# MariaPdg/thesis-fmri-reconstruction

Measured on NVIDIA B200. Metric: stage1_vaegan_train_samples_per_sec_64x64, higher is better.
Workload: dtype bf16

## Files before the change

thesis_fmri_reconstruction_b200/csrc/api.cu:

```cuda
#include <cstdarg>
#include <cstdio>
#include <cstring>
#include <cstdlib>
#include <algorithm>

#include "../../include/fmri_b200.h"
#include "simt_kernels.cuh"
#include "tc_kernels.cuh"
#include "hconv_kernels.cuh"
#include "hwgrad_kernels.cuh"
#include "cto3_kernels.cuh"
#include "mmd_kernels.cuh"
#include "eval_kernels.cuh"
#include "similarity_kernels.cuh"

using namespace fmri;

static thread_local char g_err[512] = "";
static int fail(int code, const char* fmt, ...) {
    va_list ap;
    va_start(ap, fmt);
    vsnprintf(g_err, sizeof(g_err), fmt, ap);
    va_end(ap);
    return code;
// ... 486 lines not shown
    c.num_taps = 1;
    c.lim_x = M;
    c.lim_y = 1;
    c.out_off = 0;
    c.taps[0].map = 0;
    c.taps[0].dx = 0;
    c.taps[0].dy = 0;
    c.taps[0].brow = 0;
    p.num_chunks = cdiv(K, KCH);
    p.n_total = N;
    p.n_tiles = N / BN;
    const int splits = 1;
    p.splits = splits;
    p.a_bytes = p.bw * KCH * 2;
    p.out_sn = 0;
    p.out_sy = 0;
    p.out_sx = ldc;
    p.out = Cout;
    p.out_fp32 = c_fp32;
    p.atomic_out = (splits > 1 || accumulate) ? 1 : 0;
    if (p.atomic_out && !c_fp32) return fail(FMRI_ERR_ARG, "accumulating gemm needs fp32 output");
    p.bias = bias;
    p.act = act;
    return dispatch_ig(p, BN, KCH, 1, st);
}

template <int BN, int NCH, int STAGES, int TG>
static int launch_wg(const WgParams& p, cudaStream_t st) {
    using L = WgSmem<BN, NCH, STAGES, TG>;
    static bool attr_done = false;
    if (!attr_done) {
        CUDA_OK(cudaFuncSetAttribute(wgrad_kernel<BN, NCH, STAGES, TG>, cudaFuncAttributeMaxDynamicSharedMemorySize,
                                     L::TOTAL));
        attr_done = true;
    }
    dim3 grid(cdiv(p.num_taps, TG), p.m_tiles * p.n_tiles, p.splits);
    wgrad_kernel<BN, NCH, STAGES, TG><<<grid, 192, L::TOTAL, st>>>(p);
    LAUNCH_OK();
    return 0;
}
static int wave_splits(long long base, long long max_splits) {
    const long long lo = std::max<long long>(1, (148 + base - 1) / base);
    if (max_splits <= lo) return (int)std::max<long long>(1, max_splits);
    const long long hi = std::min<long long>(max_splits, std::max<long long>(lo, (3 * 148) / base));
    long long best = lo;
    double best_score = -1.0;
    for (long long s = lo; s <= hi; ++s) {
        const long long ctas = base * s, waves = (ctas + 147) / 148;
        const double score = (double)ctas / (148.0 * waves) - 0.01 * waves;
        if (score > best_score) { best_score = score; best = s; }
    }
    return (int)best;
}
static int dispatch_wg(const WgParams& p, int BN, int NCH, cudaStream_t st) {
    if (NCH == 64 && BN == 128) return p.num_taps > 1 ? launch_wg<128, 64, 2, 2>(p, st) : launch_wg<128, 64, 3, 1>(p, st);
    if (NCH == 64 && BN == 64) return launch_wg<64, 64, 4, 1>(p, st);
    if (NCH == 32 && BN == 32) return p.num_taps % 5 == 0 ? launch_wg<32, 32, 3, 5>(p, st) : launch_wg<32, 32, 4, 1>(p, st);
    return fail(FMRI_ERR_UNSUPPORTED, "wgrad tile BN=%d NCH=%d not instantiated", BN, NCH);
}
static int run_wgrad_tc(const void* Dn, int N, int PH, int PW, int Cd, const void* Sh, int BH, int BW, int Cs,
                        int stride, int num_taps, float* ws, cudaStream_t st) {
    if (Cd % 64 || Cs % 32) return fail(FMRI_ERR_UNSUPPORTED, "wgrad tensor path needs Cd%%64==0, Cs%%32==0");
    WgParams p;
    memset(&p, 0, sizeof(p));
    pick_box(PW, PH, N, &p.bw, &p.bh, &p.bn);
    if ((p.bw * p.bh * p.bn) % 16) pick_box_pow2(PW, PH, N, &p.bw, &p.bh, &p.bn);
    p.rows = p.bw * p.bh * p.bn;
    if (p.rows % 16) return fail(FMRI_ERR_UNSUPPORTED, "wgrad pixel box %d not a multiple of 16", p.rows);
    p.tiles_x = cdiv(PW, p.bw);
    p.tiles_y = cdiv(PH, p.bh);
    p.tiles_n = cdiv(N, p.bn);
    const int NCH = (Cs % 64 == 0) ? 64 : 32;
    const int BN = (Cs % 128 == 0) ? 128 : (Cs % 64 == 0 ? 64 : 32);
    if (NCH == 32 && BN != 32) return fail(FMRI_ERR_UNSUPPORTED, "wgrad Cs=%d", Cs);
    int rc = make_act_map(&p.mapD, Dn, Cd, PW, PH, N, Cd, (long long)PW * Cd, (long long)PH * PW * Cd, 64, p.bw,
                          p.bh, p.bn);
    if (rc) return rc;
    const __nv_bfloat16* sb = reinterpret_cast<const __nv_bfloat16*>(Sh);
    if (stride == 2) {
        for (int ph = 0; ph < 2; ++ph)
            for (int pw = 0; pw < 2; ++pw) {
                const int Wp = (BW - pw + 1) / 2, Hp = (BH - ph + 1) / 2;
                rc = make_act_map(&p.mapS[ph * 2 + pw], sb + ((long long)ph * BW + pw) * Cs, Cs, Wp, Hp, N, 2LL * Cs,
                                  2LL * BW * Cs, (long long)BH * BW * Cs, NCH, p.bw, p.bh, p.bn);
                if (rc) return rc;
            }
    } else {
        rc = make_act_map(&p.mapS[0], sb, Cs, BW, BH, N, Cs, (long long)BW * Cs, (long long)BH * BW * Cs, NCH, p.bw,
                          p.bh, p.bn);
        if (rc) return rc;
    }
    p.num_taps = num_taps;
    for (int kh = 0; kh < 5; ++kh)
        for (int kw = 0; kw < 5; ++kw) {
            TapDesc& t = p.taps[kh * 5 + kw];
            if (num_taps == 1) {
                t.map = 0;
                t.dx = t.dy = 0;
            } else if (stride == 2) {
                t.map = (int16_t)((kh & 1) * 2 + (kw & 1));
                t.dy = (int16_t)((kh - 2 - (kh & 1)) / 2);
                t.dx = (int16_t)((kw - 2 - (kw & 1)) / 2);
            } else {
                t.map = 0;
                t.dy = (int16_t)(kh - 2);
                t.dx = (int16_t)(kw - 2);
            }
        }
    p.m_total = Cd;
    p.n_total = Cs;
    p.m_tiles = cdiv(Cd, 128);
    p.n_tiles = Cs / BN;
    const long long pt = (long long)p.tiles_x * p.tiles_y * p.tiles_n;
    const int tap_groups = (NCH == 32 && BN == 32 && num_taps % 5 == 0) ? num_taps / 5
                           : ((NCH == 64 && BN == 128 && num_taps > 1) ? (num_taps + 1) / 2 : num_taps);
    const long long base = (long long)tap_groups * p.m_tiles * p.n_tiles;
    p.splits = wave_splits(base, std::max<long long>(1, pt / 4));
    const long long n = (long long)num_taps * Cd * Cs;
    SCRATCH(slices, float, (long long)p.splits * n, st);
    CUDA_OK(cudaMemsetAsync(slices, 0, sizeof(float) * (size_t)p.splits * n, st));
    p.out = slices;
    p.split_stride = n;
    rc = dispatch_wg(p, BN, NCH, st);
    if (rc) return rc;
    rc = ordered_add(slices, p.splits, n, ws, st);
    CUDA_OK(cudaFreeAsync(slices, st));
    return rc;
}

extern "C" void fmri_conv_out_hw(const fmri_conv_desc* d, int* OH, int* OW) {
    if (d->transposed) {
        *OH = 2 * d->H - 1 + d->output_pad;
        *OW = 2 * d->W - 1 + d->output_pad;
    } else {
        *OH = (d->H - 1) / d->stride + 1;
        *OW = (d->W - 1) / d->stride + 1;
    }
}
static int check_conv(const fmri_conv_desc* d) {
    if (!d || d->N <= 0 || d->H <= 0 || d->W <= 0 || d->Cin <= 0 || d->Cout <= 0)
        return fail(FMRI_ERR_ARG, "bad conv descriptor");
    if (d->stride != 1 && d->stride != 2) return fail(FMRI_ERR_ARG, "conv stride must be 1 or 2");
    if (d->transposed && d->stride != 2) return fail(FMRI_ERR_ARG, "ConvTranspose2d is stride 2 only");
    if (d->dtype != FMRI_F32 && d->dtype != FMRI_BF16) return fail(FMRI_ERR_ARG, "bad dtype");
    return 0;
}
static inline long long w_so(const fmri_conv_desc* d) { return d->transposed ? 25LL : 25LL * d->Cin; }
static inline long long w_si(const fmri_conv_desc* d) { return d->transposed ? 25LL * d->Cout : 25LL; }

extern "C" size_t fmri_conv_pack_elems(const fmri_conv_desc* d) {
    size_t n = 25 * (size_t)d->Cin * d->Cout;
    const int thin = d->transposed ? d->Cout : d->Cin;
    const int other = d->transposed ? d->Cin : d->Cout;
    if (thin == 32 && d->stride == 2) n += 9 * 128 * (size_t)other;
    return n;
}

extern "C" int fmri_conv_pack_weights(const fmri_conv_desc* d, const float* w, void* pack_f, void* pack_d,
                                      void* stream) {
    int rc = check_conv(d);
    if (rc) return rc;
    const long long n = 25LL * d->Cin * d->Cout;
    if (pack_f) {
        permute4_kernel<float, __nv_bfloat16><<<grid1d(n, 256), 256, 0, S(stream)>>>(
            w, reinterpret_cast<__nv_bfloat16*>(pack_f), 1, 25, d->Cout, d->Cin, 0, 1, w_so(d), w_si(d), 0);
        LAUNCH_OK();
        if (d->transposed && d->Cout == 32 && d->stride == 2) {
            __nv_bfloat16* pk = reinterpret_cast<__nv_bfloat16*>(pack_f);
            merge_pack_kernel<<<grid1d(9LL * 128 * d->Cin, 256), 256, 0, S(stream)>>>(pk, pk + n, d->Cin);
            LAUNCH_OK();
        }
    }
    if (pack_d) {
        permute4_kernel<float, __nv_bfloat16><<<grid1d(n, 256), 256, 0, S(stream)>>>(
            w, reinterpret_cast<__nv_bfloat16*>(pack_d), 1, 25, d->Cin, d->Cout, 0, 1, w_si(d), w_so(d), 0);
        LAUNCH_OK();
// ... 142 lines not shown
    p.accumulate = accumulate;
    const float *A, *B;
    if (!d->transposed) {
        A = reinterpret_cast<const float*>(dy); p.PH = OH; p.PW = OW; p.Ca = d->Cout;
        B = reinterpret_cast<const float*>(x); p.BH = d->H; p.BW = d->W; p.Cb = d->Cin;
    } else {
        A = reinterpret_cast<const float*>(x); p.PH = d->H; p.PW = d->W; p.Ca = d->Cin;
        B = reinterpret_cast<const float*>(dy); p.BH = OH; p.BW = OW; p.Cb = d->Cout;
    }
    p.a_sn = (long long)p.PH * p.PW * p.Ca; p.a_sy = (long long)p.PW * p.Ca; p.a_sx = p.Ca; p.a_sc = 1;
    p.b_sn = (long long)p.BH * p.BW * p.Cb; p.b_sy = (long long)p.BW * p.Cb; p.b_sx = p.Cb; p.b_sc = 1;
    p.w_sa = 25LL * p.Cb;
    p.w_sb = 25;
    direct_wgrad_kernel<float, float><<<25 * p.Ca * p.Cb, 128, 0, S(stream)>>>(A, B, dw, p);
    LAUNCH_OK();
    return 0;
}

static const size_t HC_WS_PACK = 65536;
extern "C" size_t fmri_edge_workspace(const fmri_edge_desc* d) {
    return std::max(sizeof(float) * 75 * (size_t)d->C, HC_WS_PACK + (size_t)d->N * d->H * d->W * 16);
}

static bool hc_build(HcParams& p, HcPackSpec& spec, int N, int H, int W, int chunks, int stride, int OH, int OW, int BN,
                     bool flip) {
    memset(&p, 0, sizeof(p));
    memset(&spec, 0, sizeof(spec));
    p.N = N; p.H = H; p.W = W; p.chunks = chunks; p.OH = OH; p.OW = OW;
    const int hx = stride == 1 ? 4 : 2;
    if (stride == 1) {
        p.num_planes = 1;
        p.pl_ys[0] = p.pl_xs[0] = 1;
        p.pl_yoff[0] = p.pl_xoff[0] = -2;
    } else {
        p.num_planes = 4;
        for (int ph = 0; ph < 2; ++ph)
            for (int pw = 0; pw < 2; ++pw) {
                const int pl = ph * 2 + pw;
                p.pl_ys[pl] = p.pl_xs[pl] = 2;
                p.pl_yoff[pl] = ph - 2;
                p.pl_xoff[pl] = pw - 2;
            }
    }
    p.PW = OW + hx;
    if (p.PW > 200) return false;
    const int max_off = hx * p.PW + hx;
    const int nsteps = chunks >= 2 ? 25 * (chunks / 2) : 13;
    if (nsteps > HC_MAX_STEPS) return false;
    p.num_steps = nsteps;
    bool found = false;
    for (int pass = 0; pass < 2 && !found; ++pass) {
        const int mt_max = std::min(5, (pass == 0 ? 128 : 256) / BN);
        const size_t smem_cap = pass == 0 ? 110 * 1024 : 227 * 1024;
        double best = 0.0;
        for (int tht = std::min(OH, (mt_max * 128) / p.PW); tht >= 1; --tht) {
            HcParams q = p;
            q.THt = tht;
            q.tiles_y = cdiv(OH, tht);
            q.MT = cdiv((long long)tht * q.PW, 128);
            q.PH = tht + hx;
            q.slab_rows = (q.PH * q.PW + 7) / 8 * 8 + (chunks > 1 ? 2 : 0);
            const long long overshoot = ((long long)q.MT * 128 + max_off + 1 - q.slab_rows) * 16;
            if (overshoot > 0 && overshoot > hc_b_bytes(q, BN)) continue;
            if ((size_t)hc_smem_bytes(q, BN) > smem_cap) continue;
            const double eff = (double)OH * OW / ((double)q.tiles_y * q.MT * 128);
            if (eff > best + 1e-9) { best = eff; p = q; found = true; }
        }
    }
    if (!found) return false;
    int woff[25];
    for (int kh = 0; kh < 5; ++kh)
        for (int kw = 0; kw < 5; ++kw) {
            int plane = 0, dyr = kh, dxr = kw;
            if (stride == 2) {
                plane = (kh & 1) * 2 + (kw & 1);
                dyr = (kh - 2 - (kh & 1)) / 2 + 1;
                dxr = (kw - 2 - (kw & 1)) / 2 + 1;
            }
            woff[kh * 5 + kw] = plane * chunks * p.slab_rows + dyr * p.PW + dxr;
        }
    int s = 0;
    if (chunks >= 2) {
        for (int tp = 0; tp < 25; ++tp)
            for (int j = 0; j < chunks / 2; ++j, ++s) {
                p.steps[s].a_off = woff[tp] + 2 * j * p.slab_rows;
                p.steps[s].a_lbo = p.slab_rows;
                p.steps[s].b_off = s * BN;
                spec.tap[s][0] = spec.tap[s][1] = (int16_t)(flip ? 24 - tp : tp);
                spec.cb[s][0] = (int16_t)(16 * j);
                spec.cb[s][1] = (int16_t)(16 * j + 8);
            }
    } else {
        int order[25];
        for (int i = 0; i < 25; ++i) order[i] = i;
        std::sort(order, order + 25, [&](int a, int b) { return woff[a] < woff[b]; });
        {
            const int t0 = order[0];
            p.steps[s].a_off = woff[t0];
            p.steps[s].a_lbo = 1;
            p.steps[s].b_off = s * BN;
            spec.tap[s][0] = (int16_t)(flip ? 24 - t0 : t0);
            spec.tap[s][1] = -1;
            spec.cb[s][0] = spec.cb[s][1] = 0;
            ++s;
        }
        for (int i = 1; i < 25; i += 2, ++s) {
            const int t0 = order[i], t1 = order[i + 1];
            p.steps[s].a_off = woff[t0];
            p.steps[s].a_lbo = woff[t1] - woff[t0];
            p.steps[s].b_off = s * BN;
            spec.tap[s][0] = (int16_t)(flip ? 24 - t0 : t0);
            spec.tap[s][1] = (int16_t)(flip ? 24 - t1 : t1);
            spec.cb[s][0] = spec.cb[s][1] = 0;
            if (p.steps[s].a_lbo == 0) return false;
        }
    }
    return true;
}

// ... 35 lines not shown
    }
    return fail(FMRI_ERR_UNSUPPORTED, "hconv BN=%d", BN);
}

static int cto3_run(const void* X, int N, int H, int W, int C, const float* w, long long s_co, long long s_c, int flip,
                    const float* bias, int act, float* img, void* ws, cudaStream_t st) {
    if (C != 32 || W != C3_W || H < 3 || N < 74) return 1;
    C3Params p;
    memset(&p, 0, sizeof(p));
    __nv_bfloat16* wt = reinterpret_cast<__nv_bfloat16*>(ws);
    c3_pack_weights_kernel<<<cdiv(C3_NB * C, 256), 256, 0, st>>>(w, wt, s_co, s_c, flip, C);
    LAUNCH_OK();
    if (make_act_map(&p.mapX, X, C, H * W, 1, N, C, (long long)H * W * C, (long long)H * W * C, C, 128, 1, 1)) return 1;
    {
        const long long dims[2] = {C, C3_NB};
        const long long stv[1] = {C};
        const int box[2] = {C, C3_NB};
        if (make_map(&p.mapW, wt, 2, dims, stv, box, C * 2)) return 1;
    }
    p.N = N; p.H = H; p.out = img; p.bias = bias; p.act = act;
    static bool attr_done = false;
    if (!attr_done) {
        CUDA_OK(cudaFuncSetAttribute(cto3_kernel, cudaFuncAttributeMaxDynamicSharedMemorySize, C3_SMEM));
        attr_done = true;
    }
    cto3_kernel<<<std::min(N, 148), C3_THREADS, C3_SMEM, st>>>(p);
    LAUNCH_OK();
    return 0;
}

static int hconv_c_to_3(const void* X, int N, int H, int W, int C, const float* w, long long s_co, long long s_c, int flip,
                        const float* bias, int act, float* img, void* ws, cudaStream_t st) {
    if (C != 32 && C != 64) return 1;
    {
        const int rc = cto3_run(X, N, H, W, C, w, s_co, s_c, flip, bias, act, img, ws, st);
        if (rc <= 0) return rc;
    }
    HcParams p;
    HcPackSpec spec;
    if (!hc_build(p, spec, N, H, W, C / 8, 1, H, W, 16, flip != 0)) return 1;
    p.X = reinterpret_cast<const __nv_bfloat16*>(X);
    p.epi = 0; p.out = img; p.bias = bias; p.act = act; p.n_out = 3;
    return hc_run(p, spec, 16, w, 3, C, s_co, s_c, ws, st);
}

static int hconv_3_to_c(const float* i0, const float* i1, const float* i2, int nps, int N, int H, int W, int C, int stride,
                        const float* w, long long s_c, long long s_ci, int flip, const float* bias, int act, void* y,
                        void* ws, cudaStream_t st) {
    if (C != 32 && C != 64) return 1;
    const int OH = (H - 1) / stride + 1, OW = (W - 1) / stride + 1;
    HcParams p;
    HcPackSpec spec;
    if (!hc_build(p, spec, N, H, W, 1, stride, OH, OW, C, flip != 0)) return 1;
    __nv_bfloat16* img8 = reinterpret_cast<__nv_bfloat16*>(reinterpret_cast<uint8_t*>(ws) + HC_WS_PACK);
    img8_pack_kernel<<<grid1d((long long)N * H * W, 256), 256, 0, st>>>(i0, i1, i2, nps, N, (long long)H * W, img8);
    LAUNCH_OK();
    p.X = img8;
    p.epi = 1; p.out = y; p.bias = bias; p.act = act; p.n_out = C;
    return hc_run(p, spec, C, w, C, 3, s_c, s_ci, ws, st);
}

static int hwgrad_run(const void* T, const float* i0, const float* i1, const float* i2, int nps, int N, int PH, int PW, int C,
                      float* dwk, float* dbias, int flip, void* ws, cudaStream_t st, int plane = -1, int IH = 0, int IW = 0) {
    if (C != 32 && C != 64) return 1;
    HwParams p;
    memset(&p, 0, sizeof(p));
    p.N = N; p.PH = PH; p.PW = PW; p.C = C;
    p.PWp = (PW + 4 + 15) / 16 * 16;
    if (p.PWp > 128) return 1;
    const int bh_cap = 2;
    p.bh = std::max(1, std::min(std::min(PH, bh_cap), 256 / p.PWp));
    p.tiles_y = cdiv(PH, p.bh);
    p.slab_rows = ((p.bh + 4) * p.PWp + 16 + 7) / 8 * 8;
    p.d_chunk = (p.bh * p.PWp * 128 + 1023) / 1024 * 1024;
    p.stages = 2;
    if (hw_smem_bytes(p) > 227 * 1024) return 1;
    while (p.stages < HW_MAX_STAGES) {
        ++p.stages;
        if (hw_smem_bytes(p) > 110 * 1024) { --p.stages; break; }
    }
    const long long dims[4] = {C, PW, PH, N};
    const long long strides[3] = {C, (long long)PW * C, (long long)PH * PW * C};
    const int box[4] = {64, p.PWp, p.bh, 1};
    if (make_map(&p.mapT, T, 4, dims, strides, box, 128)) return 1;
    __nv_bfloat16* img8 = reinterpret_cast<__nv_bfloat16*>(reinterpret_cast<uint8_t*>(ws) + HC_WS_PACK);
    p.kh0 = 0; p.nkh = 5;
    if (plane < 0) {
        img8_pack_kernel<<<grid1d((long long)N * PH * PW, 256), 256, 0, st>>>(i0, i1, i2, nps, N, (long long)PH * PW, img8);
    } else {
        p.plane = 1; p.ph = plane >> 1; p.pw = plane & 1;
        p.kh0 = 1; p.nkh = p.ph ? 2 : 3;
        img8_plane_pack_kernel<<<grid1d((long long)N * PH * PW, 256), 256, 0, st>>>(i0, i1, i2, nps, N, IH, IW, PH, PW, p.ph,
                                                                                   p.pw, img8);
    }
    LAUNCH_OK();
    p.img8 = img8;
    p.dwk = dwk; p.dbias = dbias; p.flip = flip;
    const int smem = hw_smem_bytes(p);
    static int attr_smem = 0;
    if (smem > attr_smem) {
        CUDA_OK(cudaFuncSetAttribute(hwgrad_kernel, cudaFuncAttributeMaxDynamicSharedMemorySize, smem));
        attr_smem = smem;
    }
    const int total = N * p.tiles_y;
    const int nb = std::min(total, 148 * (smem <= 110 * 1024 ? 2 : 1));
    const long long nw = 75LL * C;
    SCRATCH(part, float, (long long)nb * (nw + C), st);
    CUDA_OK(cudaMemsetAsync(part, 0, sizeof(float) * (size_t)nb * (nw + C), st));
    p.dwk = part;
    p.dbias = dbias ? part + nb * nw : nullptr;
// ... 1088 lines not shown
```

thesis_fmri_reconstruction_b200/csrc/hconv_kernels.cuh:

```cuda
#pragma once
#include "ptx.cuh"

namespace fmri {

struct HcStep {
    uint32_t a_off;
    uint32_t a_lbo;
    uint32_t b_off;
};
constexpr int HC_MAX_STEPS = 104;

struct HcParams {
    const __nv_bfloat16* X;
    int N, H, W;
    int chunks;
    int num_planes;
    int pl_ys[4], pl_xs[4];
    int pl_yoff[4], pl_xoff[4];
    int PW, PH;
    int skip;
    int slab_rows;
    int num_steps;
    HcStep steps[HC_MAX_STEPS];
    int THt, tiles_y;
    int OH, OW;
    int MT;
    const __nv_bfloat16* Bslab;
    int epi;
    void* out;
    const float* bias;
    int act;
    int n_out;
};

__device__ __forceinline__ void cp_async16(uint32_t dst, const void* src, uint32_t src_bytes) {
    asm volatile("cp.async.cg.shared.global [%0], [%1], 16, %2;" ::"r"(dst), "l"(src), "r"(src_bytes) : "memory");
}
__device__ __forceinline__ void cp_async_wait_all() { asm volatile("cp.async.wait_all;" ::: "memory"); }

__device__ __forceinline__ void tmem_ld16(uint32_t taddr, uint32_t (&r)[16]) {
    asm volatile(
        "tcgen05.ld.sync.aligned.32x32b.x16.b32 "
        "{%0, %1, %2, %3, %4, %5, %6, %7, %8, %9, %10, %11, %12, %13, %14, %15}, [%16];"
        : "=r"(r[0]), "=r"(r[1]), "=r"(r[2]), "=r"(r[3]), "=r"(r[4]), "=r"(r[5]), "=r"(r[6]), "=r"(r[7]),
          "=r"(r[8]), "=r"(r[9]), "=r"(r[10]), "=r"(r[11]), "=r"(r[12]), "=r"(r[13]), "=r"(r[14]), "=r"(r[15])
        : "r"(taddr)
        : "memory");
}

__device__ __forceinline__ float hc_act(float v, int act) {
    if (act == 1) return fmaxf(v, 0.f);
    if (act == 2) return tanhf(v);
    if (act == 3) return 1.f / (1.f + __expf(-v));
    return v;
}

constexpr int HC_ISSUERS = 5;
constexpr int HC_PRODUCERS = 160;
constexpr int HC_EPI_WARPS = 8;
constexpr int HC_THREADS = 32 * HC_ISSUERS + HC_PRODUCERS + 32 * HC_EPI_WARPS;

__host__ __device__ inline int hc_slab_bytes(const HcParams& p) { return p.slab_rows * 16; }
__host__ __device__ inline int hc_a_buffer_bytes(const HcParams& p) { return p.num_planes * p.chunks * hc_slab_bytes(p); }
__host__ __device__ inline int hc_b_bytes(const HcParams& p, int BN) { return 2 * p.num_steps * BN * 16; }
__host__ __device__ inline int hc_smem_bytes(const HcParams& p, int BN) {
    return 2 * hc_a_buffer_bytes(p) + hc_b_bytes(p, BN) + 512 + 1024;
}

template <int BN>
__global__ void __launch_bounds__(HC_THREADS, 2) hconv_kernel(const __grid_constant__ HcParams p) {
    extern __shared__ uint8_t smem_raw[];
    uint8_t* smem = reinterpret_cast<uint8_t*>((reinterpret_cast<uintptr_t>(smem_raw) + 1023) & ~uintptr_t(1023));
    const int a_buf = hc_a_buffer_bytes(p);
    const int slab = hc_slab_bytes(p);
    const int chunks = p.chunks;
    uint8_t* sA = smem;
    uint8_t* sB = smem + 2 * a_buf;
    const int b_half = p.num_steps * BN * 16;
    uint64_t* bars = reinterpret_cast<uint64_t*>(sB + hc_b_bytes(p, BN));
    uint64_t* slab_full = bars;
    uint64_t* slab_empty = bars + 2;
    uint64_t* tmem_full = bars + 4;
    uint64_t* tmem_empty = bars + 6;
    uint64_t* b_full = bars + 8;
    uint32_t* tmem_slot = reinterpret_cast<uint32_t*>(bars + 9);
    float* s_bias = reinterpret_cast<float*>(bars + 10);

    const int warp = threadIdx.x >> 5, lane = threadIdx.x & 31;
    if (threadIdx.x < 64) s_bias[threadIdx.x] = (p.bias && p.epi == 1 && (int)threadIdx.x < BN) ? p.bias[threadIdx.x] : 0.f;
    const int total_tiles = p.N * p.tiles_y;
    const int acc_cols = p.MT * BN;
    const int issuers = p.MT < HC_ISSUERS ? p.MT : HC_ISSUERS;
    uint32_t tmem_cols = 32;
    while ((int)tmem_cols < 2 * acc_cols) tmem_cols <<= 1;

    if (threadIdx.x == 0) {
        for (int i = 0; i < 2; ++i) {
            mbar_init(&slab_full[i], HC_PRODUCERS);
            mbar_init(&slab_empty[i], issuers);
            mbar_init(&tmem_full[i], issuers);
            mbar_init(&tmem_empty[i], HC_EPI_WARPS);
        }
        mbar_init(b_full, HC_PRODUCERS);
        fence_barrier_init();
    }
    if (warp == 0) tmem_alloc(tmem_slot, tmem_cols);
    for (int i = threadIdx.x; i < (2 * a_buf) / 16; i += HC_THREADS) reinterpret_cast<uint4*>(sA)[i] = make_uint4(0u, 0u, 0u, 0u);
    fence_proxy_async_smem();
    tc_fence_before();
    __syncthreads();
    tc_fence_after();
    const uint32_t tmem_base = *tmem_slot;

    if (warp < HC_ISSUERS) {
        if (warp < issuers) {
            const uint32_t idesc = umma_idesc_bf16(128, BN, false, false);
            const uint32_t tmem_u = __shfl_sync(0xffffffffu, tmem_base, 0);
            mbar_wait(b_full, 0);
            tc_fence_after();
            const uint64_t b_base = umma_smem_desc(smem_u32(sB), b_half, 128, 0);
            int it = 0;
            for (int t = blockIdx.x; t < total_tiles; t += gridDim.x, ++it) {
                const int sb = it & 1;
                const uint32_t par = (it >> 1) & 1;
                mbar_wait(&slab_full[sb], par);
                mbar_wait(&tmem_empty[sb], par ^ 1);
                tc_fence_after();
                const uint64_t a_base = umma_smem_desc(smem_u32(sA + sb * a_buf), 0, 128, 0);
                const uint32_t d0 = tmem_u + sb * acc_cols;
                uint32_t acc = 0;
#pragma unroll 4
                for (int s = 0; s < p.num_steps; ++s) {
                    const HcStep stp = p.steps[s];
                    const uint64_t ad = (a_base | (static_cast<uint64_t>(stp.a_lbo & 0x3FFF) << 16)) + stp.a_off;
                    const uint64_t bd = b_base + stp.b_off;
                    if (p.skip & 4) continue;
                    for (int m = warp; m < p.MT; m += issuers)
                        umma_bf16_elect(d0 + m * BN, ad + (uint32_t)(m * 128), bd, idesc, acc);
                    acc = 1;
                }
                umma_commit_elect(&slab_empty[sb]);
                umma_commit_elect(&tmem_full[sb]);
            }
        }
        __syncwarp();
    } else if (warp < HC_ISSUERS + HC_PRODUCERS / 32) {
        const int ptid = threadIdx.x - 32 * HC_ISSUERS;
        {
            const int n16 = hc_b_bytes(p, BN) / 16;
            const uint32_t b0 = smem_u32(sB);
            for (int i = ptid; i < n16; i += HC_PRODUCERS)
                cp_async16(b0 + i * 16, reinterpret_cast<const uint8_t*>(p.Bslab) + (size_t)i * 16, 16);
            cp_async_wait_all();
            fence_proxy_async_smem();
            mbar_arrive(b_full);
        }
        const int halo_px = p.PH * p.PW;
        const int Cx = chunks * 8;
        int it = 0;
        for (int t = blockIdx.x; t < total_tiles; t += gridDim.x, ++it) {
            const int sb = it & 1;
            const uint32_t par = (it >> 1) & 1;
            const int n = t / p.tiles_y;
            const int oy0 = (t - n * p.tiles_y) * p.THt;
            mbar_wait(&slab_empty[sb], par ^ 1);
            const uint32_t a0 = smem_u32(sA + sb * a_buf);
            const __nv_bfloat16* Xn = p.X + (size_t)n * p.H * p.W * Cx;
            for (int pl = 0; pl < ((p.skip & 1) ? 0 : p.num_planes); ++pl) {
                const int ys = p.pl_ys[pl], xs = p.pl_xs[pl], yo = p.pl_yoff[pl], xo = p.pl_xoff[pl];
                const uint32_t pbase = a0 + pl * chunks * slab;
                const int j = ptid % chunks;
                const int row_step = HC_PRODUCERS / chunks;
                int row = ptid / chunks;
                int sy = row / p.PW, sx = row - sy * p.PW;
                const uint32_t dst0 = pbase + j * slab;
                for (; row < halo_px; row += row_step) {
                    const int iy = (oy0 + sy) * ys + yo, ix = sx * xs + xo;
                    const bool ok = iy >= 0 && iy < p.H && ix >= 0 && ix < p.W;
                    const __nv_bfloat16* src = ok ? Xn + ((size_t)iy * p.W + ix) * Cx + j * 8 : Xn;
                    cp_async16(dst0 + row * 16, src, ok ? 16u : 0u);
                    sx += row_step;
                    while (sx >= p.PW) { sx -= p.PW; ++sy; }
                }
            }
            cp_async_wait_all();
            fence_proxy_async_smem();
            mbar_arrive(&slab_full[sb]);
        }
    } else {
        const int q = warp & 3;
        const int egrp = (warp - (HC_ISSUERS + HC_PRODUCERS / 32)) >> 2;
        int it = 0;
        for (int t = blockIdx.x; t < total_tiles; t += gridDim.x, ++it) {
            const int sb = it & 1;
            const uint32_t par = (it >> 1) & 1;
            const int n = t / p.tiles_y;
            const int oy0 = (t - n * p.tiles_y) * p.THt;
            mbar_wait(&tmem_full[sb], par);
            tc_fence_after();
            for (int m = egrp; m < p.MT; m += HC_EPI_WARPS / 4) {
                const int r = m * 128 + q * 32 + lane;
                const int yy = r / p.PW, xx = r - yy * p.PW;
                const bool valid = yy < p.THt && (oy0 + yy) < p.OH && xx < p.OW && !(p.skip & 2);
                const uint32_t tad = tmem_base + (static_cast<uint32_t>(q * 32) << 16) + sb * acc_cols + m * BN;
                if (p.epi == 0) {
                    uint32_t v[16];
                    tmem_ld16(tad, v);
                    tmem_ld_wait();
                    if (valid) {
                        float* o = reinterpret_cast<float*>(p.out) + (((size_t)n * p.n_out) * p.OH + (oy0 + yy)) * p.OW + xx;
                        const size_t cs = (size_t)p.OH * p.OW;
#pragma unroll
                        for (int c = 0; c < 16; ++c) {
                            if (c < p.n_out) {
                                const float f = __uint_as_float(v[c]) + (p.bias ? __ldg(p.bias + c) : 0.f);
                                o[c * cs] = hc_act(f, p.act);
                            }
                        }
                    }
                } else {
                    __nv_bfloat16* o = reinterpret_cast<__nv_bfloat16*>(p.out) +
                                       (((size_t)n * p.OH + (oy0 + yy)) * p.OW + xx) * BN;
#pragma unroll 1
                    for (int c0 = 0; c0 < BN; c0 += 16) {
                        uint32_t v[16];
                        tmem_ld16(tad + c0, v);
                        tmem_ld_wait();
                        float f[16];
#pragma unroll
                        for (int c = 0; c < 16; ++c) f[c] = __uint_as_float(v[c]);
                        if (p.bias) {
#pragma unroll
                            for (int c = 0; c < 16; ++c) f[c] += s_bias[c0 + c];
                        }
                        if (p.act == 1) {
#pragma unroll
                            for (int c = 0; c < 16; ++c) f[c] = fmaxf(f[c], 0.f);
                        } else if (p.act != 0) {
#pragma unroll
                            for (int c = 0; c < 16; ++c) f[c] = hc_act(f[c], p.act);
                        }
                        uint32_t pk[8];
#pragma unroll
                        for (int c = 0; c < 8; ++c) pk[c] = pack_bf16x2(f[2 * c], f[2 * c + 1]);
                        if (valid) {
                            *reinterpret_cast<uint4*>(o + c0) = make_uint4(pk[0], pk[1], pk[2], pk[3]);
                            *reinterpret_cast<uint4*>(o + c0 + 8) = make_uint4(pk[4], pk[5], pk[6], pk[7]);
                        }
                    }
                }
            }
            tc_fence_before();
            __syncwarp();
            if (lane == 0) mbar_arrive(&tmem_empty[sb]);
        }
    }
    tc_fence_before();
    __syncthreads();
    tc_fence_after();
    if (warp == 0) tmem_dealloc(tmem_base, tmem_cols);
}

struct HcPackSpec {
    int16_t tap[HC_MAX_STEPS][2];
    int16_t cb[HC_MAX_STEPS][2];
};
__global__ void hc_pack_weights_kernel(const float* __restrict__ w, __nv_bfloat16* __restrict__ dst,
                                       const __grid_constant__ HcPackSpec spec, int num_steps, int BN, int n_real,
                                       int c_real, long long s_n, long long s_c) {
    const int rows = num_steps * BN;
    const int total = 2 * rows * 8;
    for (int i = blockIdx.x * blockDim.x + threadIdx.x; i < total; i += gridDim.x * blockDim.x) {
// ... 49 lines not shown
```

thesis_fmri_reconstruction_b200/csrc/tc_kernels.cuh:

```cuda
#pragma once
#include "ptx.cuh"

namespace fmri {

struct TapDesc {
    int16_t map;
    int16_t dx;
    int16_t dy;
    int16_t ncol;
    int32_t brow;
};

struct TapClass {
    int num_taps;
    int lim_x, lim_y;
    long long out_off;
    TapDesc taps[25];
};

enum { ACT_NONE = 0, ACT_RELU = 1, ACT_TANH = 2, ACT_SIGMOID = 3 };

struct IgParams {
    CUtensorMap mapA[4];
    CUtensorMap mapB;
// ... 806 lines not shown
                        if (!SMEM_STATS && do_stats) {
#pragma unroll
                            for (int j = 0; j < 16; ++j) {
                                f[2 * j] = __uint_as_float(pk[j] << 16);
                                f[2 * j + 1] = __uint_as_float(pk[j] & 0xffff0000u);
                            }
                        }
                    }
                    if (!SMEM_STATS && do_stats) {
                        float g2[32];
#pragma unroll
                        for (int j = 0; j < 32; ++j) {
                            f[j] = valid ? f[j] : 0.f;
                            g2[j] = f[j] * f[j];
                        }
#pragma unroll
                        for (int j = 0; j < 32; ++j) {
                            sacc[j] += f[j];
                            qacc[j] += g2[j];
                        }
                        pending = true;
                    }
                }
                if (!SMEM_STATS && do_stats && pending && !p.merge) {
                    const float s1 = warp_colsum32(sacc, lane);
                    const float s2 = warp_colsum32(qacc, lane);
                    my_stat[c0 + lane] += s1;
                    my_stat[BN + c0 + lane] += s2;
#pragma unroll
                    for (int j = 0; j < 32; ++j) sacc[j] = qacc[j] = 0.f;
                    pending = false;
                }
            }
            if (!SMEM_STATS && do_stats && pending) {
                const float s1 = warp_colsum32(sacc, lane);
                const float s2 = warp_colsum32(qacc, lane);
                my_stat[lane] += s1;
                my_stat[BN + lane] += s2;
            }
            tc_fence_before();
            __syncwarp();
            if (lane == 0) mbar_arrive(&tempty[buf]);
            if (do_stats) ++stat_cnt;
            ++lt;
        }
        if (do_stats && stat_cnt > 0) flush_stats(stat_nt);
    }
    tc_fence_before();
    __syncthreads();
    tc_fence_after();
    if (warp == 1) tmem_dealloc(tmem_base, TMEM_COLS);
}

struct WgParams {
    CUtensorMap mapD;
    CUtensorMap mapS[4];
    TapDesc taps[25];
    int num_taps;
    int rows;
    float* out;
    long long split_stride;
    int bw, bh, bn;
    int tiles_x, tiles_y, tiles_n;
    int m_total, n_total;
    int m_tiles, n_tiles;
    int splits;
};

template <int BN, int NCH, int STAGES, int TG = 1>
struct WgSmem {
    static constexpr int D_BYTES = 128 * 128 * 2;
    static constexpr int S_BYTES = 128 * BN * 2;
    static constexpr int STAGE_BYTES = D_BYTES + TG * S_BYTES;
    static constexpr int BAR_OFF = STAGES * STAGE_BYTES;
    static constexpr int TOTAL = BAR_OFF + (2 * STAGES + 1) * 8 + 16 + 1024;
};

template <int BN, int NCH, int STAGES, int TG>
__global__ void __launch_bounds__(192) wgrad_kernel(const __grid_constant__ WgParams p) {
    using L = WgSmem<BN, NCH, STAGES, TG>;
    extern __shared__ uint8_t smem_raw[];
    uint8_t* smem = reinterpret_cast<uint8_t*>((reinterpret_cast<uintptr_t>(smem_raw) + 1023) & ~uintptr_t(1023));
    uint64_t* full_bar = reinterpret_cast<uint64_t*>(smem + L::BAR_OFF);
    uint64_t* empty_bar = full_bar + STAGES;
    uint64_t* tmem_full = empty_bar + STAGES;
    uint32_t* tmem_slot = reinterpret_cast<uint32_t*>(tmem_full + 1);

    const int warp = threadIdx.x >> 5;
    const int lane = threadIdx.x & 31;
    const int tap0 = blockIdx.x * TG;
    const int tg_live = min(TG, p.num_taps - tap0);
    const int mtile = blockIdx.y % p.m_tiles;
    const int ntile = blockIdx.y / p.m_tiles;
    const int split = blockIdx.z;
    const int pt_total = p.tiles_x * p.tiles_y * p.tiles_n;
    const int pt_begin = (int)((long long)split * pt_total / p.splits);
    const int pt_end = (int)((long long)(split + 1) * pt_total / p.splits);
    if (pt_begin >= pt_end) return;
    const int npt = pt_end - pt_begin;

    constexpr uint32_t TMEM_COLS = (TG * BN) <= 32 ? 32 : ((TG * BN) <= 64 ? 64 : ((TG * BN) <= 128 ? 128 : ((TG * BN) <= 256 ? 256 : 512)));
    static_assert(TG * BN <= 512, "accumulators must fit TMEM");
    constexpr int S_CHUNKS = BN / NCH;
    const uint32_t d_chunk_bytes = p.rows * 128;
    const uint32_t s_chunk_bytes = p.rows * NCH * 2;

    if (warp == 0 && lane == 0) {
        tma_prefetch_desc(&p.mapD);
        tma_prefetch_desc(&p.mapS[p.taps[tap0].map]);
        for (int s = 0; s < STAGES; ++s) {
// ... 62 lines not shown
                const uint64_t adesc = umma_smem_desc(sd, d_chunk_bytes, 8 * 128, UMMA_SW128);
                if constexpr (TG > 1 && BN == NCH && TG * BN <= 256) {
                    const uint32_t idesc_m = umma_idesc_bf16(128, tg_live * BN, true, true);
                    const uint64_t bdesc = umma_smem_desc(sd + L::D_BYTES, L::S_BYTES, 8 * s_row, s_layout);
                    for (int k = 0; k < ksteps; ++k)
                        umma_bf16_elect(tmem_u, adesc + ((k * 16 * 128) >> 4), bdesc + ((k * 16 * s_row) >> 4), idesc_m,
                                        (i | k) != 0);
                } else {
#pragma unroll
                    for (int tg = 0; tg < TG; ++tg) {
                        if (tg >= tg_live) break;
                        const uint64_t bdesc =
                            umma_smem_desc(sd + L::D_BYTES + tg * L::S_BYTES, s_chunk_bytes, 8 * s_row, s_layout);
                        for (int k = 0; k < ksteps; ++k)
                            umma_bf16_elect(tmem_u + tg * BN, adesc + ((k * 16 * 128) >> 4),
                                            bdesc + ((k * 16 * s_row) >> 4), idesc, (i | k) != 0);
                    }
                }
                umma_commit_elect(&empty_bar[st]);
            }
            umma_commit_elect(tmem_full);
        }
        __syncwarp();
    } else {
        mbar_wait(tmem_full, 0);
        tc_fence_after();
        const int q = warp & 3;
        const int m = mtile * 128 + q * 32 + lane;
        const bool valid = m < p.m_total;
#pragma unroll 1
        for (int tg = 0; tg < tg_live; ++tg) {
            float* orow = p.out + blockIdx.z * p.split_stride + ((long long)(tap0 + tg) * p.m_total + m) * p.n_total +
                          ntile * BN;
#pragma unroll 1
            for (int c0 = 0; c0 < BN; c0 += 32) {
                uint32_t v[32];
                tmem_ld32(tmem_base + (static_cast<uint32_t>(q * 32) << 16) + tg * BN + c0, v);
                tmem_ld_wait();
                if (valid) {
#pragma unroll
                    for (int j = 0; j < 32; j += 4)
                        red_add_v4(orow + c0 + j, __uint_as_float(v[j]), __uint_as_float(v[j + 1]),
                                   __uint_as_float(v[j + 2]), __uint_as_float(v[j + 3]));
                }
            }
        }
        tc_fence_before();
    }
    __syncthreads();
    tc_fence_after();
    if (warp == 1) tmem_dealloc(tmem_base, TMEM_COLS);
}

}
```

Baseline: 40910.

## Fuse RGB image packing into hconv producer and stage BN=64 epilogue through smem

Drops the separate img8 pack kernel and has the conv producers read fp32 RGB planes directly, convert them to bf16 and store them into the A slab. For BN=64 it also adds a per-warp shared-memory staging buffer so epilogue outputs are written as coalesced 16-byte rows, and it changes the tile-height heuristic to minimise tiles*(MT+1) instead of maximising efficiency. The aim is to save a kernel launch plus a global round-trip and to improve store coalescing. The cost is synchronous loads in the producer path instead of cp.async, and a little more shared memory.

```diff
diff --git a/thesis_fmri_reconstruction_b200/csrc/api.cu b/thesis_fmri_reconstruction_b200/csrc/api.cu
--- a/thesis_fmri_reconstruction_b200/csrc/api.cu
+++ b/thesis_fmri_reconstruction_b200/csrc/api.cu
@@ -880,7 +880,7 @@
     for (int pass = 0; pass < 2 && !found; ++pass) {
         const int mt_max = std::min(5, (pass == 0 ? 128 : 256) / BN);
         const size_t smem_cap = pass == 0 ? 110 * 1024 : 227 * 1024;
-        double best = 0.0;
+        long long best = 0;
         for (int tht = std::min(OH, (mt_max * 128) / p.PW); tht >= 1; --tht) {
             HcParams q = p;
             q.THt = tht;
@@ -891,8 +891,8 @@
             const long long overshoot = ((long long)q.MT * 128 + max_off + 1 - q.slab_rows) * 16;
             if (overshoot > 0 && overshoot > hc_b_bytes(q, BN)) continue;
             if ((size_t)hc_smem_bytes(q, BN) > smem_cap) continue;
-            const double eff = (double)OH * OW / ((double)q.tiles_y * q.MT * 128);
-            if (eff > best + 1e-9) { best = eff; p = q; found = true; }
+            const long long cost = (long long)q.tiles_y * (q.MT + 1);
+            if (!found || cost < best) { best = cost; p = q; found = true; }
         }
     }
     if (!found) return false;
@@ -1034,10 +1034,7 @@
     HcParams p;
     HcPackSpec spec;
     if (!hc_build(p, spec, N, H, W, 1, stride, OH, OW, C, flip != 0)) return 1;
-    __nv_bfloat16* img8 = reinterpret_cast<__nv_bfloat16*>(reinterpret_cast<uint8_t*>(ws) + HC_WS_PACK);
-    img8_pack_kernel<<<grid1d((long long)N * H * W, 256), 256, 0, st>>>(i0, i1, i2, nps, N, (long long)H * W, img8);
-    LAUNCH_OK();
-    p.X = img8;
+    p.img[0] = i0; p.img[1] = i1; p.img[2] = i2; p.n_per_src = nps;
     p.epi = 1; p.out = y; p.bias = bias; p.act = act; p.n_out = C;
     return hc_run(p, spec, C, w, C, 3, s_c, s_ci, ws, st);
 }
diff --git a/thesis_fmri_reconstruction_b200/csrc/hconv_kernels.cuh b/thesis_fmri_reconstruction_b200/csrc/hconv_kernels.cuh
--- a/thesis_fmri_reconstruction_b200/csrc/hconv_kernels.cuh
+++ b/thesis_fmri_reconstruction_b200/csrc/hconv_kernels.cuh
@@ -12,6 +12,8 @@
 
 struct HcParams {
     const __nv_bfloat16* X;
+    const float* img[3];
+    int n_per_src;
     int N, H, W;
     int chunks;
     int num_planes;
@@ -48,6 +50,9 @@
         : "memory");
 }
 
+__device__ __forceinline__ void hc_tmem_ld(uint32_t taddr, uint32_t (&r)[16]) { tmem_ld16(taddr, r); }
+__device__ __forceinline__ void hc_tmem_ld(uint32_t taddr, uint32_t (&r)[32]) { tmem_ld32(taddr, r); }
+
 __device__ __forceinline__ float hc_act(float v, int act) {
     if (act == 1) return fmaxf(v, 0.f);
     if (act == 2) return tanhf(v);
@@ -63,8 +68,13 @@
 __host__ __device__ inline int hc_slab_bytes(const HcParams& p) { return p.slab_rows * 16; }
 __host__ __device__ inline int hc_a_buffer_bytes(const HcParams& p) { return p.num_planes * p.chunks * hc_slab_bytes(p); }
 __host__ __device__ inline int hc_b_bytes(const HcParams& p, int BN) { return 2 * p.num_steps * BN * 16; }
+constexpr int HC_STAGE_LINE = 144;
+__host__ __device__ inline int hc_stage_bytes(int BN) { return BN == 64 ? HC_EPI_WARPS * (32 * BN * 2 / 128) * HC_STAGE_LINE : 0; }
+__host__ __device__ inline int hc_stage_offset(const HcParams& p, int BN) {
+    return 2 * hc_a_buffer_bytes(p) + hc_b_bytes(p, BN) + 512;
+}
 __host__ __device__ inline int hc_smem_bytes(const HcParams& p, int BN) {
-    return 2 * hc_a_buffer_bytes(p) + hc_b_bytes(p, BN) + 512 + 1024;
+    return hc_stage_offset(p, BN) + hc_stage_bytes(BN) + 1024;
 }
 
 template <int BN>
@@ -85,6 +95,7 @@
     uint64_t* b_full = bars + 8;
     uint32_t* tmem_slot = reinterpret_cast<uint32_t*>(bars + 9);
     float* s_bias = reinterpret_cast<float*>(bars + 10);
+    uint8_t* s_stage = smem + hc_stage_offset(p, BN);
 
     const int warp = threadIdx.x >> 5, lane = threadIdx.x & 31;
     if (threadIdx.x < 64) s_bias[threadIdx.x] = (p.bias && p.epi == 1 && (int)threadIdx.x < BN) ? p.bias[threadIdx.x] : 0.f;
@@ -166,6 +177,11 @@
             mbar_wait(&slab_empty[sb], par ^ 1);
             const uint32_t a0 = smem_u32(sA + sb * a_buf);
             const __nv_bfloat16* Xn = p.X + (size_t)n * p.H * p.W * Cx;
+            const int si = p.img[0] ? n / p.n_per_src : 0;
+            const float* im = p.img[0] ? (si == 0 ? p.img[0] : (si == 1 ? p.img[1] : p.img[2])) +
+                                             (size_t)(n - si * p.n_per_src) * 3 * p.H * p.W
+                                       : nullptr;
+            const size_t HW = (size_t)p.H * p.W;
             for (int pl = 0; pl < ((p.skip & 1) ? 0 : p.num_planes); ++pl) {
                 const int ys = p.pl_ys[pl], xs = p.pl_xs[pl], yo = p.pl_yoff[pl], xo = p.pl_xoff[pl];
                 const uint32_t pbase = a0 + pl * chunks * slab;
@@ -174,6 +190,27 @@
                 int row = ptid / chunks;
                 int sy = row / p.PW, sx = row - sy * p.PW;
                 const uint32_t dst0 = pbase + j * slab;
+                if (im) {
+                    for (; row < halo_px; row += 4 * row_step) {
+                        uint32_t a[4], b[4];
+#pragma unroll
+                        for (int k = 0; k < 4; ++k) {
+                            const int iy = (oy0 + sy) * ys + yo, ix = sx * xs + xo;
+                            a[k] = b[k] = 0u;
+                            if (row + k * row_step < halo_px && iy >= 0 && iy < p.H && ix >= 0 && ix < p.W) {
+                                const float* q = im + (size_t)iy * p.W + ix;
+                                a[k] = pack_bf16x2(__ldg(q), __ldg(q + HW));
+                                b[k] = pack_bf16x2(__ldg(q + 2 * HW), 0.f);
+                            }
+                            sx += row_step;
+                            while (sx >= p.PW) { sx -= p.PW; ++sy; }
+                        }
+#pragma unroll
+                        for (int k = 0; k < 4; ++k)
+                            if (row + k * row_step < halo_px) sts_v4(dst0 + (row + k * row_step) * 16, a[k], b[k], 0u, 0u);
+                    }
+                    continue;
+                }
                 for (; row < halo_px; row += row_step) {
                     const int iy = (oy0 + sy) * ys + yo, ix = sx * xs + xo;
                     const bool ok = iy >= 0 && iy < p.H && ix >= 0 && ix < p.W;
@@ -189,7 +226,9 @@
         }
     } else {
         const int q = warp & 3;
-        const int egrp = (warp - (HC_ISSUERS + HC_PRODUCERS / 32)) >> 2;
+        const int ewarp = warp - (HC_ISSUERS + HC_PRODUCERS / 32);
+        const int egrp = ewarp >> 2;
+        const uint32_t stage_u32 = smem_u32(s_stage) + ewarp * (hc_stage_bytes(BN) / HC_EPI_WARPS);
         int it = 0;
         for (int t = blockIdx.x; t < total_tiles; t += gridDim.x, ++it) {
             const int sb = it & 1;
@@ -218,6 +257,56 @@
                             }
                         }
                     }
+                } else if constexpr (BN == 64) {
+                    constexpr int LPR = BN / 8;
+                    constexpr int RPL = 128 / (2 * BN);
+                    const uint32_t stg = stage_u32 + (lane / RPL) * HC_STAGE_LINE + (lane % RPL) * (2 * BN);
+                    constexpr int CW = 32;
+#pragma unroll
+                    for (int c0 = 0; c0 < BN; c0 += CW) {
+                        uint32_t v[CW];
+                        if (!(p.skip & 8)) {
+                            hc_tmem_ld(tad + c0, v);
+                            tmem_ld_wait();
+                        } else {
+#pragma unroll
+                            for (int c = 0; c < CW; ++c) v[c] = 0u;
+                        }
+                        float f[CW];
+#pragma unroll
+                        for (int c = 0; c < CW; ++c) f[c] = __uint_as_float(v[c]);
+                        if (p.bias) {
+#pragma unroll
+                            for (int c = 0; c < CW; ++c) f[c] += s_bias[c0 + c];
+                        }
+                        if (p.act == 1) {
+#pragma unroll
+                            for (int c = 0; c < CW; ++c) f[c] = fmaxf(f[c], 0.f);
+                        } else if (p.act != 0) {
+#pragma unroll
+                            for (int c = 0; c < CW; ++c) f[c] = hc_act(f[c], p.act);
+                        }
+#pragma unroll
+                        for (int j = 0; j < CW / 8; ++j)
+                            sts_v4(stg + (c0 + 8 * j) * 2, pack_bf16x2(f[8 * j], f[8 * j + 1]),
+                                   pack_bf16x2(f[8 * j + 2], f[8 * j + 3]), pack_bf16x2(f[8 * j + 4], f[8 * j + 5]),
+                                   pack_bf16x2(f[8 * j + 6], f[8 * j + 7]));
+                    }
+                    const uint32_t vmask = __ballot_sync(0xffffffffu, valid);
+                    const int pix = (oy0 + yy) * p.OW + xx;
+                    __nv_bfloat16* out_n = reinterpret_cast<__nv_bfloat16*>(p.out) + (size_t)n * p.OH * p.OW * BN;
+                    __syncwarp();
+                    constexpr int RPI = 32 / LPR;
+                    const int piece = lane % LPR;
+                    const uint32_t ldb = stage_u32 + (lane / LPR / RPL) * HC_STAGE_LINE + (lane / LPR % RPL) * (2 * BN) + piece * 16;
+#pragma unroll
+                    for (int j = 0; j < LPR; ++j) {
+                        const int rr = j * RPI + lane / LPR;
+                        const int pr = __shfl_sync(0xffffffffu, pix, rr);
+                        const uint4 v4 = lds_v4(ldb + (j * RPI / RPL) * HC_STAGE_LINE);
+                        if ((vmask >> rr) & 1u) *reinterpret_cast<uint4*>(out_n + (size_t)pr * BN + piece * 8) = v4;
+                    }
+                    __syncwarp();
                 } else {
                     __nv_bfloat16* o = reinterpret_cast<__nv_bfloat16*>(p.out) +
                                        (((size_t)n * p.OH + (oy0 + yy)) * p.OW + xx) * BN;
```

Result: no change. 40890, median of 6 (-0.1%).

## Add column-grouped wgrad kernel sharing one tall source tile across vertical taps

Applied to the files above, without the earlier changes.

Adds a persistent-style weight-gradient kernel that groups conv taps sharing the same map and dx with consecutive dy. For each group it loads one vertically extended source tile and reuses it for up to three tap accumulators in TMEM. It also packs several work units per CTA. The aim is to cut redundant TMA loads of the shifted source activations. It is used only when a wave-count heuristic favors it, and it adds serialized unit processing per CTA with a single accumulator buffer.

```diff
diff --git a/thesis_fmri_reconstruction_b200/csrc/api.cu b/thesis_fmri_reconstruction_b200/csrc/api.cu
--- a/thesis_fmri_reconstruction_b200/csrc/api.cu
+++ b/thesis_fmri_reconstruction_b200/csrc/api.cu
@@ -562,6 +562,53 @@
     }
     return (int)best;
 }
+template <int BN, int STAGES>
+static int launch_wg_col(const WgParams& p, int ctas, cudaStream_t st) {
+    using L = WgColSmem<BN, STAGES>;
+    static bool attr_done = false;
+    if (!attr_done) {
+        CUDA_OK(cudaFuncSetAttribute(wgrad_col_kernel<BN, STAGES>, cudaFuncAttributeMaxDynamicSharedMemorySize, L::TOTAL));
+        attr_done = true;
+    }
+    wgrad_col_kernel<BN, STAGES><<<ctas, 192, L::TOTAL, st>>>(p);
+    LAUNCH_OK();
+    return 0;
+}
+static int tap_columns(WgParams& p) {
+    int n = 0;
+    bool used[25] = {};
+    for (int t = 0; t < p.num_taps; ++t) {
+        if (used[t]) continue;
+        WgGroup g{};
+        for (int u = t; u < p.num_taps; ++u) {
+            const TapDesc &a = p.taps[t], &b = p.taps[u];
+            if (used[u] || a.map != b.map || a.dx != b.dx) continue;
+            if (g.num == WG_COL_TAPS) return 0;
+            int j = g.num++;
+            for (; j > 0 && p.taps[g.tap[j - 1]].dy > b.dy; --j) g.tap[j] = g.tap[j - 1];
+            g.tap[j] = (int8_t)u;
+            used[u] = true;
+        }
+        for (int j = 1; j < g.num; ++j)
+            if (p.taps[g.tap[j]].dy != p.taps[g.tap[0]].dy + j) return 0;
+        p.groups[n++] = g;
+    }
+    std::stable_sort(p.groups, p.groups + n, [](const WgGroup& a, const WgGroup& b) { return a.num > b.num; });
+    for (int c = 0, g = 0; c < 4; ++c) {
+        while (g < n && p.groups[g].num > WG_COL_TAPS - c) ++g;
+        p.col_class[c] = (int8_t)g;
+    }
+    return n;
+}
+static long long col_ctas(const WgParams& p) {
+    long long ctas = 0;
+    for (int c = 0; c < WG_COL_TAPS; ++c) {
+        const long long units = (long long)(p.col_class[c + 1] - p.col_class[c]) * p.m_tiles * p.n_tiles * p.splits;
+        const int upc = WG_COL_PACK / (WG_COL_TAPS - c);
+        ctas += (units + upc - 1) / upc;
+    }
+    return ctas;
+}
 static int dispatch_wg(const WgParams& p, int BN, int NCH, cudaStream_t st) {
     if (NCH == 64 && BN == 128) return p.num_taps > 1 ? launch_wg<128, 64, 2, 2>(p, st) : launch_wg<128, 64, 3, 1>(p, st);
     if (NCH == 64 && BN == 64) return launch_wg<64, 64, 4, 1>(p, st);
@@ -583,23 +630,6 @@
     const int NCH = (Cs % 64 == 0) ? 64 : 32;
     const int BN = (Cs % 128 == 0) ? 128 : (Cs % 64 == 0 ? 64 : 32);
     if (NCH == 32 && BN != 32) return fail(FMRI_ERR_UNSUPPORTED, "wgrad Cs=%d", Cs);
-    int rc = make_act_map(&p.mapD, Dn, Cd, PW, PH, N, Cd, (long long)PW * Cd, (long long)PH * PW * Cd, 64, p.bw,
-                          p.bh, p.bn);
-    if (rc) return rc;
-    const __nv_bfloat16* sb = reinterpret_cast<const __nv_bfloat16*>(Sh);
-    if (stride == 2) {
-        for (int ph = 0; ph < 2; ++ph)
-            for (int pw = 0; pw < 2; ++pw) {
-                const int Wp = (BW - pw + 1) / 2, Hp = (BH - ph + 1) / 2;
-                rc = make_act_map(&p.mapS[ph * 2 + pw], sb + ((long long)ph * BW + pw) * Cs, Cs, Wp, Hp, N, 2LL * Cs,
-                                  2LL * BW * Cs, (long long)BH * BW * Cs, NCH, p.bw, p.bh, p.bn);
-                if (rc) return rc;
-            }
-    } else {
-        rc = make_act_map(&p.mapS[0], sb, Cs, BW, BH, N, Cs, (long long)BW * Cs, (long long)BH * BW * Cs, NCH, p.bw,
-                          p.bh, p.bn);
-        if (rc) return rc;
-    }
     p.num_taps = num_taps;
     for (int kh = 0; kh < 5; ++kh)
         for (int kw = 0; kw < 5; ++kw) {
@@ -626,12 +656,36 @@
                            : ((NCH == 64 && BN == 128 && num_taps > 1) ? (num_taps + 1) / 2 : num_taps);
     const long long base = (long long)tap_groups * p.m_tiles * p.n_tiles;
     p.splits = wave_splits(base, std::max<long long>(1, pt / 4));
+    int col_grid = 0;
+    if (NCH == 64 && BN == 128 && num_taps > 1 && p.bn == 1 && p.bw % 8 == 0 && (p.bw * p.bh) % 16 == 0 &&
+        p.bn * p.bw * (p.bh + WG_COL_TAPS - 1) <= WG_COL_MAX_PX && tap_columns(p) > 0) {
+        const long long ctas = col_ctas(p), ctas_tg2 = (long long)(num_taps + 1) / 2 * p.m_tiles * p.n_tiles * p.splits;
+        if (WG_COL_PACK * cdiv(ctas, 148LL) <= 2 * cdiv(ctas_tg2, 148LL)) col_grid = (int)ctas;
+    }
+    const int s_bh = col_grid ? p.bh + WG_COL_TAPS - 1 : p.bh;
+    int rc = make_act_map(&p.mapD, Dn, Cd, PW, PH, N, Cd, (long long)PW * Cd, (long long)PH * PW * Cd, 64, p.bw,
+                          p.bh, p.bn);
+    if (rc) return rc;
+    const __nv_bfloat16* sb = reinterpret_cast<const __nv_bfloat16*>(Sh);
+    if (stride == 2) {
+        for (int ph = 0; ph < 2; ++ph)
+            for (int pw = 0; pw < 2; ++pw) {
+                const int Wp = (BW - pw + 1) / 2, Hp = (BH - ph + 1) / 2;
+                rc = make_act_map(&p.mapS[ph * 2 + pw], sb + ((long long)ph * BW + pw) * Cs, Cs, Wp, Hp, N, 2LL * Cs,
+                                  2LL * BW * Cs, (long long)BH * BW * Cs, NCH, p.bw, s_bh, p.bn);
+                if (rc) return rc;
+            }
+    } else {
+        rc = make_act_map(&p.mapS[0], sb, Cs, BW, BH, N, Cs, (long long)BW * Cs, (long long)BH * BW * Cs, NCH, p.bw,
+                          s_bh, p.bn);
+        if (rc) return rc;
+    }
     const long long n = (long long)num_taps * Cd * Cs;
     SCRATCH(slices, float, (long long)p.splits * n, st);
     CUDA_OK(cudaMemsetAsync(slices, 0, sizeof(float) * (size_t)p.splits * n, st));
     p.out = slices;
     p.split_stride = n;
-    rc = dispatch_wg(p, BN, NCH, st);
+    rc = col_grid ? launch_wg_col<128, 3>(p, col_grid, st) : dispatch_wg(p, BN, NCH, st);
     if (rc) return rc;
     rc = ordered_add(slices, p.splits, n, ws, st);
     CUDA_OK(cudaFreeAsync(slices, st));
diff --git a/thesis_fmri_reconstruction_b200/csrc/tc_kernels.cuh b/thesis_fmri_reconstruction_b200/csrc/tc_kernels.cuh
--- a/thesis_fmri_reconstruction_b200/csrc/tc_kernels.cuh
+++ b/thesis_fmri_reconstruction_b200/csrc/tc_kernels.cuh
@@ -882,10 +882,20 @@
     if (warp == 1) tmem_dealloc(tmem_base, TMEM_COLS);
 }
 
+struct WgGroup {
+    int8_t num;
+    int8_t tap[3];
+};
+constexpr int WG_COL_TAPS = 3;
+constexpr int WG_COL_MAX_PX = 160;
+constexpr int WG_COL_PACK = 6;
+
 struct WgParams {
     CUtensorMap mapD;
     CUtensorMap mapS[4];
     TapDesc taps[25];
+    WgGroup groups[25];
+    int8_t col_class[4];
     int num_taps;
     int rows;
     float* out;
@@ -1054,4 +1064,177 @@
     if (warp == 1) tmem_dealloc(tmem_base, TMEM_COLS);
 }
 
+template <int BN, int STAGES>
+struct WgColSmem {
+    static constexpr int D_BYTES = 128 * 128 * 2;
+    static constexpr int STAGE_BYTES = D_BYTES + WG_COL_MAX_PX * BN * 2;
+    static constexpr int BAR_OFF = STAGES * STAGE_BYTES;
+    static constexpr int TOTAL = BAR_OFF + (2 * STAGES + 2) * 8 + 16 + 1024;
+};
+
+__device__ __forceinline__ bool wg_col_unit(const WgParams& p, int cta, int j, int& grp, int& mn, int& split) {
+    const int per_split = p.m_tiles * p.n_tiles;
+    for (int c = 0; c < WG_COL_TAPS; ++c) {
+        const int gc = p.col_class[c + 1] - p.col_class[c];
+        const int units = gc * per_split * p.splits;
+        const int upc = WG_COL_PACK / (WG_COL_TAPS - c);
+        const int ctas = (units + upc - 1) / upc;
+        if (cta < ctas) {
+            const int u = cta + j * ctas;
+            if (j >= upc || u >= units) return false;
+            split = u / (gc * per_split);
+            const int l = u % (gc * per_split);
+            grp = p.col_class[c] + l % gc;
+            mn = l / gc;
+            return true;
+        }
+        cta -= ctas;
+    }
+    return false;
 }
+
+template <int BN, int STAGES>
+__global__ void __launch_bounds__(192) wgrad_col_kernel(const __grid_constant__ WgParams p) {
+    constexpr int NCH = 64, S_CHUNKS = BN / NCH;
+    using L = WgColSmem<BN, STAGES>;
+    extern __shared__ uint8_t smem_raw[];
+    uint8_t* smem = reinterpret_cast<uint8_t*>((reinterpret_cast<uintptr_t>(smem_raw) + 1023) & ~uintptr_t(1023));
+    uint64_t* full_bar = reinterpret_cast<uint64_t*>(smem + L::BAR_OFF);
+    uint64_t* empty_bar = full_bar + STAGES;
+    uint64_t* tfull = empty_bar + STAGES;
+    uint64_t* tempty = tfull + 1;
+    uint32_t* tmem_slot = reinterpret_cast<uint32_t*>(tempty + 1);
+
+    const int warp = threadIdx.x >> 5;
+    const int lane = threadIdx.x & 31;
+    const int pt_total = p.tiles_x * p.tiles_y * p.tiles_n;
+    constexpr uint32_t TMEM_COLS = WG_COL_TAPS * BN <= 256 ? 256 : 512;
+    static_assert(WG_COL_TAPS * BN <= 512, "accumulators must fit TMEM");
+    const uint32_t d_chunk_bytes = p.rows * 128;
+    const uint32_t s_chunk_bytes = p.bn * p.bw * (p.bh + WG_COL_TAPS - 1) * NCH * 2;
+
+    if (warp == 0 && lane == 0) {
+        tma_prefetch_desc(&p.mapD);
+        for (int m = 0; m < 4; ++m) tma_prefetch_desc(&p.mapS[m]);
+        for (int s = 0; s < STAGES; ++s) {
+            mbar_init(&full_bar[s], 1);
+            mbar_init(&empty_bar[s], 1);
+        }
+        mbar_init(tfull, 1);
+        mbar_init(tempty, 4);
+        fence_barrier_init();
+    }
+    if (warp == 1) tmem_alloc(tmem_slot, TMEM_COLS);
+    tc_fence_before();
+    __syncthreads();
+    tc_fence_after();
+    const uint32_t tmem_base = *tmem_slot;
+
+    int grp, mn, split;
+    if (warp == 0) {
+        int it = 0;
+        for (int j = 0; wg_col_unit(p, blockIdx.x, j, grp, mn, split); ++j) {
+            const TapDesc t0 = p.taps[p.groups[grp].tap[0]];
+            const int mtile = mn % p.m_tiles, ntile = mn / p.m_tiles;
+            const int pt_begin = (int)((long long)split * pt_total / p.splits);
+            const int pt_end = (int)((long long)(split + 1) * pt_total / p.splits);
+            const int d_chunks_live = (p.m_total - mtile * 128) >= 128 ? 2 : 1;
+            const uint32_t tx_bytes = d_chunks_live * d_chunk_bytes + S_CHUNKS * s_chunk_bytes;
+            int tx = pt_begin % p.tiles_x;
+            int ty = (pt_begin / p.tiles_x) % p.tiles_y;
+            int tn = pt_begin / (p.tiles_x * p.tiles_y);
+            for (int i = pt_begin; i < pt_end; ++i, ++it) {
+                const int st = it % STAGES;
+                mbar_wait(&empty_bar[st], ((it / STAGES) & 1) ^ 1);
+                mbar_arrive_expect_tx_elect(&full_bar[st], tx_bytes);
+                const int x0 = tx * p.bw, y0 = ty * p.bh, n0 = tn * p.bn;
+                uint8_t* sd = smem + st * L::STAGE_BYTES;
+                for (int cchunk = 0; cchunk < d_chunks_live; ++cchunk)
+                    tma_load_4d_elect(sd + cchunk * d_chunk_bytes, &p.mapD, &full_bar[st], mtile * 128 + cchunk * 64, x0,
+                                      y0, n0);
+#pragma unroll
+                for (int cchunk = 0; cchunk < S_CHUNKS; ++cchunk)
+                    tma_load_4d_elect(sd + L::D_BYTES + cchunk * s_chunk_bytes, &p.mapS[t0.map], &full_bar[st],
+                                      ntile * BN + cchunk * NCH, x0 + t0.dx, y0 + t0.dy, n0);
+                if (++tx == p.tiles_x) {
+                    tx = 0;
+                    if (++ty == p.tiles_y) {
+                        ty = 0;
+                        ++tn;
+                    }
+                }
+            }
+        }
+        __syncwarp();
+    } else if (warp == 1) {
+        constexpr uint32_t idesc = umma_idesc_bf16(128, BN, true, true);
+        constexpr uint32_t s_row = NCH * 2;
+        const uint32_t tmem_u = __shfl_sync(0xffffffffu, tmem_base, 0);
+        const int img_px = p.bw * p.bh, tall_px = p.bw * (p.bh + WG_COL_TAPS - 1);
+        int it = 0;
+        for (int j = 0; wg_col_unit(p, blockIdx.x, j, grp, mn, split); ++j) {
+            const int tg_live = p.groups[grp].num;
+            const int npt = (int)((long long)(split + 1) * pt_total / p.splits) -
+                            (int)((long long)split * pt_total / p.splits);
+            if (j > 0) {
+                mbar_wait(tempty, (j - 1) & 1);
+                tc_fence_after();
+            }
+            for (int i = 0; i < npt; ++i, ++it) {
+                const int st = it % STAGES;
+                mbar_wait(&full_bar[st], (it / STAGES) & 1);
+                tc_fence_after();
+                const uint32_t sd = smem_u32(smem + st * L::STAGE_BYTES);
+                const uint64_t adesc = umma_smem_desc(sd, d_chunk_bytes, 8 * 128, UMMA_SW128);
+                const uint64_t bdesc = umma_smem_desc(sd + L::D_BYTES, s_chunk_bytes, 8 * s_row, UMMA_SW128);
+#pragma unroll 1
+                for (int tg = 0; tg < tg_live; ++tg) {
+                    int k = 0;
+                    for (int n = 0; n < p.bn; ++n)
+                        for (int r = 0; r < img_px; r += 16, ++k) {
+                            const uint32_t spx = n * tall_px + tg * p.bw + r;
+                            umma_bf16_elect(tmem_u + tg * BN, adesc + ((k * 16 * 128) >> 4),
+                                            bdesc + ((spx * s_row) >> 4), idesc, (i | k) != 0);
+                        }
+                }
+                umma_commit_elect(&empty_bar[st]);
+            }
+            umma_commit_elect(tfull);
+        }
+        __syncwarp();
+    } else {
+        const int q = warp & 3;
+        for (int j = 0; wg_col_unit(p, blockIdx.x, j, grp, mn, split); ++j) {
+            const int mtile = mn % p.m_tiles, ntile = mn / p.m_tiles;
+            const int m = mtile * 128 + q * 32 + lane;
+            const bool valid = m < p.m_total;
+            mbar_wait(tfull, j & 1);
+            tc_fence_after();
+#pragma unroll 1
+            for (int tg = 0; tg < p.groups[grp].num; ++tg) {
+                float* orow = p.out + split * p.split_stride +
+                              ((long long)p.groups[grp].tap[tg] * p.m_total + m) * p.n_total + ntile * BN;
+#pragma unroll 1
+                for (int c0 = 0; c0 < BN; c0 += 32) {
+                    uint32_t v[32];
+                    tmem_ld32(tmem_base + (static_cast<uint32_t>(q * 32) << 16) + tg * BN + c0, v);
+                    tmem_ld_wait();
+                    if (valid) {
+#pragma unroll
+                        for (int jj = 0; jj < 32; jj += 4)
+                            red_add_v4(orow + c0 + jj, __uint_as_float(v[jj]), __uint_as_float(v[jj + 1]),
+                                       __uint_as_float(v[jj + 2]), __uint_as_float(v[jj + 3]));
+                    }
+                }
+            }
+            tc_fence_before();
+            __syncwarp();
+            if (lane == 0) mbar_arrive(tempty);
+        }
+    }
+    __syncthreads();
+    tc_fence_after();
+    if (warp == 1) tmem_dealloc(tmem_base, TMEM_COLS);
+}
+
+}
```

Result: faster. 40510 before, 40960 after, median of 6 (+1.1%).
